# Oneflow-Inc/libai

Measured on AMD Instinct MI355X. Metric: tokens/sec (whole node), GPT-2 345M 3D-parallel at 1/2/4/8 MI355X, higher is better.
Workload: dtype bf16; 1 GPU; model=gpt2-345m (nl24 h1024 nah16 seq1024), global_batch=48, seq_len=1024, parallelism=dp1

## Files before the change

### libai_amd/csrc/kernels/flash_attn.hip

```cpp
#include "common.h"
#include "launchers.h"

#include <type_traits>

namespace {

typedef __bf16 bf16_t;
typedef __bf16 bf16x8_t __attribute__((ext_vector_type(8)));
typedef __bf16 bf16x4_t __attribute__((ext_vector_type(4)));
typedef float f32x16_t __attribute__((ext_vector_type(16)));

#define QB 32
#define NW 4
#define QBLK (QB * NW)
#define KVB 64

#ifdef FLASH_SETPRIO
#define PRIO_HI() __builtin_amdgcn_s_setprio(1)
#define PRIO_LO() __builtin_amdgcn_s_setprio(0)
#else
#define PRIO_HI()
#define PRIO_LO()
#endif

__device__ __forceinline__ uint32_t pack_bf16x2(float lo, float hi) {
  union {
    uint32_t u;
    bf16_t h[2];
  } r;
  r.h[0] = (bf16_t)lo;
  r.h[1] = (bf16_t)hi;
  return r.u;
}

__device__ __forceinline__ float and_f32(float x, uint32_t m) {
  return __uint_as_float(__float_as_uint(x) & m);
}

__device__ __forceinline__ float mul_then_sub(float a, float b, float c) {
#pragma clang fp contract(off)
  return a * b - c;
}

__device__ __forceinline__ bf16x8_t repack_chunk(const float* sv8) {
  uint32_t x0 = pack_bf16x2(sv8[0], sv8[1]);
  uint32_t z0 = pack_bf16x2(sv8[2], sv8[3]);
  uint32_t y0 = pack_bf16x2(sv8[4], sv8[5]);
  uint32_t w0 = pack_bf16x2(sv8[6], sv8[7]);
  auto rx = __builtin_amdgcn_permlane32_swap(x0, y0, false, false);
  auto rz = __builtin_amdgcn_permlane32_swap(z0, w0, false, false);
  uint32_t words[4] = {(uint32_t)rx[0], (uint32_t)rz[0], (uint32_t)rx[1],
                       (uint32_t)rz[1]};
  bf16x8_t out;
  memcpy(&out, words, 16);
  return out;
}


template <int D>
__device__ __forceinline__ void row_img_write(bf16_t* lds, int row, int col8,
                                              bf16x8_t val) {
  int byte = (row * D + col8 * 8) * 2;
  byte ^= (row & 15) << 4;
  *(bf16x8_t*)((char*)lds + byte) = val;
}

template <int D>
__device__ __forceinline__ bf16x8_t row_img_frag(const bf16_t* lds, int row, int c,
                                                 int hi) {
  int byte = (row * D + c * 16 + hi * 8) * 2;
  byte ^= (row & 15) << 4;
  return *(const bf16x8_t*)((const char*)lds + byte);
}

template <int D>
__device__ __forceinline__ void tr_img_write(bf16_t* lds, int row, int d0,
                                             bf16x8_t val) {
  int idx = (((row >> 2) * (D / 16) + (d0 >> 4)) * 64) + (row & 3) * 16 + (d0 & 15);
  *(bf16x8_t*)(lds + idx) = val;
}

template <int D>
__device__ __forceinline__ bf16x8_t tr_img_frag(const bf16_t* lds, int rbase, int dt,
                                                int lane) {
  const int hi = lane >> 5;
  const int l31 = lane & 31;
  const int r0 = rbase + hi * 8;
  const int d0 = dt * 32 + (l31 & ~15);
  const bf16_t* p0 =
      lds + (((r0 >> 2) * (D / 16) + (d0 >> 4)) * 64) + (lane & 15) * 4;
  const bf16_t* p1 =
      lds + ((((r0 + 4) >> 2) * (D / 16) + (d0 >> 4)) * 64) + (lane & 15) * 4;
  bf16x4_t a = __builtin_amdgcn_ds_read_tr16_b64_v4bf16(
      (__attribute__((address_space(3))) bf16x4_t*)p0);
  bf16x4_t b = __builtin_amdgcn_ds_read_tr16_b64_v4bf16(
      (__attribute__((address_space(3))) bf16x4_t*)p1);
  bf16x8_t out;
#pragma unroll
  for (int j = 0; j < 4; ++j) {
    out[j] = a[j];
    out[4 + j] = b[j];
  }
  return out;
}

template <int ROWS, int D, bool ROW_IMG, bool TR_IMG>
__device__ __forceinline__ void stage_tile(bf16_t* row_lds, bf16_t* tr_lds,
                                           const bf16_t* gp, int row0, int bound,
                                           int64_t stride, int tid) {
  constexpr int CHUNKS_TOTAL = ROWS * D / 8;
  constexpr int ITER = CDIV(CHUNKS_TOTAL, 256);
#pragma unroll
  for (int cc = 0; cc < ITER; ++cc) {
    const int flat = tid + cc * 256;
    if (flat >= CHUNKS_TOTAL) break;
    const int row = flat / (D / 8);
    const int col8 = flat % (D / 8);
    const int gr = row0 + row;
    bf16x8_t val =
        (gr < bound) ? *(const bf16x8_t*)(gp + (int64_t)gr * stride + col8 * 8)
                     : bf16x8_t{};
    if (ROW_IMG) row_img_write<D>(row_lds, row, col8, val);
    if (TR_IMG) tr_img_write<D>(tr_lds, row, col8 * 8, val);
  }
}

__device__ __forceinline__ uint32_t drop_hash4(uint64_t seed, uint64_t bh,
                                               int64_t Sq, int64_t Sk4, int q,
                                               int kv4) {
  (void)Sq;
  return rnd_hash2(seed, (uint32_t)q * (uint32_t)Sk4 + (uint32_t)kv4,
                   (uint32_t)bh);
}

__device__ __forceinline__ float drop_keep_byte(uint32_t h4, int kv_lo,
                                                uint32_t thr8, float ks) {
  return (((h4 >> (kv_lo * 8)) & 0xFFu) >= thr8) ? ks : 0.f;
}

__device__ __forceinline__ float drop_keep(uint64_t seed, uint64_t bh, int64_t Sq,
                                           int64_t Sk, int q, int kv, uint32_t thr8,
                                           float ks) {
  uint32_t h = drop_hash4(seed, bh, Sq, Sk >> 2, q, kv >> 2);
  return drop_keep_byte(h, kv & 3, thr8, ks);
}

__device__ __forceinline__ int block_tile() {
  return (int)((blockIdx.x + blockIdx.y) % gridDim.x);
}

__device__ __forceinline__ int doc_lo_load(const int* __restrict__ row, int i,
                                           int S) {
  return min(max(row[min(i, S - 1)], 0), i);
}

__device__ __forceinline__ int doc_hi_load(const int* __restrict__ row, int i,
                                           int S) {
  return min(max(row[min(i, S - 1)], i + 1), S);
}

#define RELB_LOG2E 1.4426950408889634f

__device__ __forceinline__ float relb_load(const float* __restrict__ row, int t,
                                           int n_diag) {
  return row[min(max(t, 0), n_diag - 1)];
}

#define RELB_RING 256

__device__ __forceinline__ void relb_flush(float* ring, float* __restrict__ grow,
                                           int tid, int count, int a0, int t_off,
                                           int n_diag) {
  if (tid < count) {
    const int a = a0 + tid;
    const float g = ring[a & (RELB_RING - 1)];
    ring[a & (RELB_RING - 1)] = 0.f;
    const int t = a + t_off;
    if (g != 0.f && t >= 0 && t < n_diag) atomicAdd(grow + t, g);
  }
}

template <int D, FlashVariant V>
__global__ __launch_bounds__(256, D == 64 ? 3 : 2) void flash_fwd_kernel(
    const bf16_t* __restrict__ q, const bf16_t* __restrict__ k,
    const bf16_t* __restrict__ v, bf16_t* __restrict__ o, float* __restrict__ lse,
    const int* __restrict__ kv_len, int64_t q_sb, int64_t q_ss, int64_t q_sh,
    int64_t k_sb, int64_t k_ss, int64_t k_sh, int64_t v_sb, int64_t v_ss,
    int64_t v_sh, int64_t o_sb, int64_t o_ss, int64_t o_sh, int H, int Sq, int Sk,
    float scale, float p_drop, uint64_t seed, int causal, int kv_group,
    const float* __restrict__ alibi_slopes, int window,
    const float* __restrict__ rel_bias, const int* __restrict__ doc_start) {
  constexpr bool ALIBI = V == FlashVariant::kAlibi,
                 WINDOW = V == FlashVariant::kWindow,
                 RELB = V == FlashVariant::kRelBias, DOCS = V == FlashVariant::kDocs;
  constexpr int DT = D / 32;
  constexpr int KC = D / 16;

  __shared__ __align__(16) bf16_t k_lds[2 * KVB * D];
  __shared__ __align__(16) bf16_t v_lds[2 * KVB * D];
  constexpr int FWD_DIAGS = 2 * KVB + QBLK - 1;
  __shared__ float rb_lds[RELB ? FWD_DIAGS : 1];

  const int tid = threadIdx.x;
  const int wave = tid >> 6;
  const int lane = tid & 63;
  const int l31 = lane & 31;
  const int hi = lane >> 5;

  const int bh = blockIdx.y;
  const int b = bh / H, h = bh % H;
  const int q_block = block_tile() * QBLK;
  const int q_base = __builtin_amdgcn_readfirstlane(q_block + wave * QB);

  const int hk = h / kv_group;
  const bf16_t* qp = q + b * q_sb + h * q_sh;
  const bf16_t* kp = k + b * k_sb + hk * k_sh;
  const bf16_t* vp = v + b * v_sb + hk * v_sh;

  const float qscale = scale * 1.4426950408889634f;
  bf16x8_t qfrag[KC];
  {
    const int qrow = min(q_base + l31, Sq - 1);
#pragma unroll
    for (int c = 0; c < KC; ++c) {
      bf16x8_t raw = *(const bf16x8_t*)(qp + (int64_t)qrow * q_ss + c * 16 + hi * 8);
#pragma unroll
      for (int j = 0; j < 8; ++j) raw[j] = (bf16_t)((float)raw[j] * qscale);
      qfrag[c] = raw;
    }
  }

  f32x16_t oacc[DT];
#pragma unroll
  for (int t = 0; t < DT; ++t) oacc[t] = f32x16_t{};
  float m_run = -3.0e38f, l_run = 0.f;

  const int sk_eff = (kv_len != nullptr) ? kv_len[b] : Sk;
  const int kv_end = causal ? min(sk_eff, q_block + QBLK) : sk_eff;
  const int n_rounds = CDIV(kv_end, 2 * KVB);
  const float ks = (p_drop > 0.f) ? 1.0f / (1.0f - p_drop) : 1.0f;
  const int qg = q_base + l31;
  float slope2 = 0.f;
  if constexpr (ALIBI) slope2 = alibi_slopes[h] * 1.4426950408889634f;

  int round0 = 0;
  if constexpr (WINDOW) round0 = max(0, q_block - window + 1) / (2 * KVB);
  int doc_lo = 0, doc_lo_w = 0, doc_lo_top = 0;
  if constexpr (DOCS) {
    const int* dsp = doc_start + (int64_t)b * Sq;
    doc_lo = doc_lo_load(dsp, qg, Sq);
    round0 = __builtin_amdgcn_readfirstlane(doc_lo_load(dsp, q_block, Sq)) /
             (2 * KVB);
    doc_lo_w = __builtin_amdgcn_readfirstlane(doc_lo_load(dsp, q_base, Sq));
    doc_lo_top =
        __builtin_amdgcn_readfirstlane(doc_lo_load(dsp, q_base + QB - 1, Sq));
  }
  const int n_diag = Sq + Sk - 1;
  const float* rbp = nullptr;
  if constexpr (RELB) rbp = rel_bias + (int64_t)h * n_diag;
  const int rb_lane = (QBLK - 1) - (qg - q_block);

  for (int round = round0; round < n_rounds; ++round) {
    const int kvR = round * 2 * KVB;
    __syncthreads();
    stage_tile<2 * KVB, D, true, false>(k_lds, nullptr, kp, kvR, Sk, k_ss, tid);
    stage_tile<2 * KVB, D, false, true>(nullptr, v_lds, vp, kvR, Sk, v_ss, tid);
    if constexpr (RELB) {
      if (tid < FWD_DIAGS)
        rb_lds[tid] =
            relb_load(rbp, kvR - q_block - (QBLK - 1) + tid + (Sq - 1), n_diag) *
            RELB_LOG2E;
    }
    __syncthreads();

    for (int sub = 0; sub < 2; ++sub) {
    const int kv0 = kvR + sub * KVB;
    const int ro = sub * KVB;
    if (kv0 >= kv_end || (causal && kv0 > q_base + QB - 1)) continue;
    if constexpr (WINDOW) {
      if (kv0 + KVB - 1 < q_base - window + 1) continue;
    }
    if constexpr (DOCS) {
      if (kv0 + KVB - 1 < doc_lo_w) continue;
    }

    f32x16_t s0{}, s1{};
    PRIO_HI();
#pragma unroll
    for (int c = 0; c < KC; ++c) {
      bf16x8_t ka = row_img_frag<D>(k_lds, ro + l31, c, hi);
      s0 = __builtin_amdgcn_mfma_f32_32x32x16_bf16(ka, qfrag[c], s0, 0, 0, 0);
      bf16x8_t kb = row_img_frag<D>(k_lds, ro + l31 + 32, c, hi);
      s1 = __builtin_amdgcn_mfma_f32_32x32x16_bf16(kb, qfrag[c], s1, 0, 0, 0);
    }
    PRIO_LO();

    float sv[2][16];
    bool interior = kv0 + KVB <= sk_eff && q_base + QB <= Sq &&
                    (!causal || q_base >= kv0 + KVB - 1);
    if constexpr (WINDOW) interior = interior && (q_base + QB - 1 - kv0 < window);
    if constexpr (DOCS) interior = interior && (kv0 >= doc_lo_top);
    auto softmax_tile = [&](auto masked_c) {
      constexpr bool MASKED = decltype(masked_c)::value;
      float pmax = -3.0e38f;
      float rel0 = 0.f;
      if constexpr (ALIBI) rel0 = (float)(kv0 + 4 * hi - qg);
#pragma unroll
      for (int r = 0; r < 16; ++r) {
        int kva = kv0 + (r & 3) + 8 * (r >> 2) + 4 * hi;
        int kvb = kva + 32;
        float a = s0[r], bb = s1[r];
        if constexpr (ALIBI) {
          const float off = (float)((r & 3) + 8 * (r >> 2));
          a = fmaf(slope2, rel0 + off, a);
          bb = fmaf(slope2, rel0 + (off + 32.f), bb);
        }
        if constexpr (RELB) {
          const int e = rb_lane + ro + (r & 3) + 8 * (r >> 2) + 4 * hi;
          a += rb_lds[e];
          bb += rb_lds[e + 32];
        }
        if constexpr (MASKED) {
          if (kva >= sk_eff || (causal && kva > qg)) a = -3.0e38f;
          if (kvb >= sk_eff || (causal && kvb > qg)) bb = -3.0e38f;
          if constexpr (WINDOW) {
            if (qg - kva >= window) a = -3.0e38f;
            if (qg - kvb >= window) bb = -3.0e38f;
          }
          if constexpr (DOCS) {
            if (kva < doc_lo) a = -3.0e38f;
            if (kvb < doc_lo) bb = -3.0e38f;
          }
        }
        sv[0][r] = a;
        sv[1][r] = bb;
        pmax = fmaxf(pmax, fmaxf(a, bb));
      }
      pmax = fmaxf(pmax, __shfl_xor(pmax, 32));

      const float m_new = fmaxf(m_run, pmax);
      float alpha = __builtin_amdgcn_exp2f(m_run - m_new);
      if constexpr (MASKED) alpha = (m_run <= -3.0e38f) ? 0.f : alpha;
      m_run = m_new;
      float lsum = 0.f;
#pragma unroll
      for (int t = 0; t < 2; ++t)
#pragma unroll
        for (int r = 0; r < 16; ++r) {
          float e = __builtin_amdgcn_exp2f(sv[t][r] - m_new);
          if constexpr (MASKED) e = (sv[t][r] <= -3.0e38f) ? 0.f : e;
          sv[t][r] = e;
          lsum += e;
        }
      lsum += __shfl_xor(lsum, 32);
      l_run = l_run * alpha + lsum;
      return alpha;
    };
    const float alpha = interior ? softmax_tile(std::false_type{})
                                 : softmax_tile(std::true_type{});
#pragma unroll
    for (int t = 0; t < DT; ++t)
#pragma unroll
      for (int r = 0; r < 16; ++r) oacc[t][r] *= alpha;

    if (p_drop > 0.f) {
      const uint32_t thr8 = drop_threshold_u8(p_drop);
#pragma unroll
      for (int t = 0; t < 2; ++t)
#pragma unroll
        for (int r4 = 0; r4 < 4; ++r4) {
          const int kvb = kv0 + t * 32 + 8 * r4 + 4 * hi;
          const uint32_t h = drop_hash4(seed, bh, Sq, Sk >> 2, qg, kvb >> 2);
#pragma unroll
          for (int j = 0; j < 4; ++j)
            sv[t][r4 * 4 + j] *= drop_keep_byte(h, j, thr8, ks);
        }
    }

    PRIO_HI();
#pragma unroll
    for (int t = 0; t < 2; ++t) {
#pragma unroll
      for (int c16 = 0; c16 < 2; ++c16) {
        bf16x8_t pfrag = repack_chunk(&sv[t][c16 * 8]);
        const int kvc = t * 32 + c16 * 16;
#pragma unroll
        for (int dt = 0; dt < DT; ++dt) {
          bf16x8_t vfrag = tr_img_frag<D>(v_lds, ro + kvc, dt, lane);
          oacc[dt] =
              __builtin_amdgcn_mfma_f32_32x32x16_bf16(vfrag, pfrag, oacc[dt], 0, 0, 0);
        }
      }
    }
    PRIO_LO();
    }
  }

  const float inv_l = (l_run > 0.f) ? 1.0f / l_run : 0.f;
  bf16_t* op = o + b * o_sb + h * o_sh + (int64_t)qg * o_ss;
  if (qg < Sq) {
#pragma unroll
    for (int dt = 0; dt < DT; ++dt)
#pragma unroll
      for (int r4 = 0; r4 < 4; ++r4) {
        bf16x4_t pk;
#pragma unroll
        for (int j = 0; j < 4; ++j) pk[j] = (bf16_t)(oacc[dt][r4 * 4 + j] * inv_l);
        *(bf16x4_t*)(op + dt * 32 + 8 * r4 + 4 * hi) = pk;
      }
    if (hi == 0 && lse != nullptr)
      lse[((int64_t)bh * Sq) + qg] =
          m_run * 0.6931471805599453f + __logf(l_run > 0.f ? l_run : 1.f);
  }
}

template <int D>
__global__ void rowdot_kernel(const bf16_t* __restrict__ dout,
                              const bf16_t* __restrict__ o, float* __restrict__ drow,
                              int64_t sb, int64_t ss, int64_t sh, int H, int Sq,
                              int64_t nrows) {
  constexpr int LPR = D / 8;
  constexpr int RPW = 64 / LPR;
  const int64_t wave_id = ((int64_t)blockIdx.x * blockDim.x + threadIdx.x) / 64;
  const int lane = threadIdx.x & 63;
  const int64_t row = wave_id * RPW + lane / LPR;
  if (row >= nrows) return;
  const int64_t BSH = (int64_t)Sq * H;
  const int64_t b = row / BSH;
  const int64_t rem = row % BSH;
  const int64_t qi = rem / H;
  const int64_t h = rem % H;
  const bf16_t* dp = dout + b * sb + qi * ss + h * sh + (lane % LPR) * 8;
  const bf16_t* op = o + b * sb + qi * ss + h * sh + (lane % LPR) * 8;
  u16x8 dv = *(const u16x8*)dp;
  u16x8 ov = *(const u16x8*)op;
  float s = 0.f;
#pragma unroll
  for (int j = 0; j < 8; ++j) s += bf2f(dv[j]) * bf2f(ov[j]);
#pragma unroll
  for (int off = LPR / 2; off > 0; off >>= 1) s += __shfl_xor(s, off, 64);
  if (lane % LPR == 0) drow[(b * H + h) * Sq + qi] = s;
}

template <int D, FlashVariant V>
__global__ __launch_bounds__(256, 2) void flash_bwd_kv_kernel(
    const bf16_t* __restrict__ q, const bf16_t* __restrict__ k,
    const bf16_t* __restrict__ v, const bf16_t* __restrict__ dout,
    const float* __restrict__ lse, const float* __restrict__ drow,
    const int* __restrict__ kv_len, bf16_t* __restrict__ dk,
    bf16_t* __restrict__ dv, int64_t q_sb, int64_t q_ss,
    int64_t q_sh, int64_t k_sb, int64_t k_ss, int64_t k_sh, int64_t v_sb,
    int64_t v_ss, int64_t v_sh, int64_t do_sb, int64_t do_ss, int64_t do_sh,
    int64_t dk_sb, int64_t dk_ss, int64_t dk_sh, int64_t dv_sb, int64_t dv_ss,
    int64_t dv_sh, int H, int Sq, int Sk, float scale, float p_drop, uint64_t seed,
    int causal, int kv_group, const float* __restrict__ alibi_slopes,
    int window, const float* __restrict__ rel_bias,
    const int* __restrict__ doc_end) {
  constexpr bool ALIBI = V == FlashVariant::kAlibi,
                 WINDOW = V == FlashVariant::kWindow,
                 RELB = V == FlashVariant::kRelBias, DOCS = V == FlashVariant::kDocs;
  constexpr int DT = D / 32;
  constexpr int KC = D / 16;
  constexpr int QTILE = (D == 64) ? 2 * QB : QB;
  constexpr int NSUB = QTILE / QB;
  constexpr int KV_DIAGS = QBLK + QTILE - 1;
  __shared__ float rb_lds[RELB ? KV_DIAGS : 1];

  __shared__ __align__(16) bf16_t q_row[QTILE * D];
  __shared__ __align__(16) bf16_t q_tr[QTILE * D];
  __shared__ __align__(16) bf16_t do_row[QTILE * D];
  __shared__ __align__(16) bf16_t do_tr[QTILE * D];
  __shared__ __align__(16) float lse_lds[QTILE];
  __shared__ __align__(16) float drow_lds[QTILE];
  constexpr bool PIPE = D == 64;

  const int tid = threadIdx.x;
  const int wave = tid >> 6;
  const int lane = tid & 63;
  const int l31 = lane & 31;
  const int hi = lane >> 5;

  const int Hkv = H / kv_group;
  const int bhk = blockIdx.y;
  const int b = bhk / Hkv, hk = bhk % Hkv;
  const int kv_block = block_tile() * QBLK;
  const int kv_base = __builtin_amdgcn_readfirstlane(kv_block + wave * QB);
  const int kvg = kv_base + l31;

  const bf16_t* kp = k + b * k_sb + hk * k_sh;
  const bf16_t* vp = v + b * v_sb + hk * v_sh;

  constexpr bool KV_PERSIST = D == 64;
  const int kvr_ld = min(kvg, Sk - 1);
  auto load_kf = [&](int c) {
    return *(const bf16x8_t*)(kp + (int64_t)kvr_ld * k_ss + c * 16 + hi * 8);
  };
  auto load_vf = [&](int c) {
    return *(const bf16x8_t*)(vp + (int64_t)kvr_ld * v_ss + c * 16 + hi * 8);
  };
  bf16x8_t kf[KV_PERSIST ? KC : 1], vf[KV_PERSIST ? KC : 1];
  if constexpr (KV_PERSIST) {
#pragma unroll
    for (int c = 0; c < KC; ++c) {
      kf[c] = load_kf(c);
      vf[c] = load_vf(c);
    }
  }
  auto get_kf = [&](int c) {
    if constexpr (KV_PERSIST) return kf[c];
    else return load_kf(c);
  };
  auto get_vf = [&](int c) {
    if constexpr (KV_PERSIST) return vf[c];
    else return load_vf(c);
  };

  f32x16_t dk_acc[DT], dv_acc[DT];
#pragma unroll
  for (int t = 0; t < DT; ++t) {
    dk_acc[t] = f32x16_t{};
    dv_acc[t] = f32x16_t{};
  }

  const float ks = (p_drop > 0.f) ? 1.0f / (1.0f - p_drop) : 1.0f;
  const int sk_eff = (kv_len != nullptr) ? kv_len[b] : Sk;
  const int qt_start = causal ? (kv_block / QTILE) : 0;
  int q_hi = Sq;
  if constexpr (WINDOW) q_hi = min(Sq, kv_block + QBLK + window - 1);
  int doc_hi = 0, doc_hi_w = 0, doc_hi_bot = 0;
  if constexpr (DOCS) {
    const int* dep = doc_end + (int64_t)b * Sk;
    doc_hi = doc_hi_load(dep, kvg, Sk);
    const int k_last = max(min(kv_block + QBLK, min(Sk, sk_eff)) - 1, 0);
    q_hi = min(Sq, __builtin_amdgcn_readfirstlane(doc_hi_load(dep, k_last, Sk)));
    doc_hi_w =
        __builtin_amdgcn_readfirstlane(doc_hi_load(dep, kv_base + QB - 1, Sk));
    doc_hi_bot = __builtin_amdgcn_readfirstlane(doc_hi_load(dep, kv_base, Sk));
  }
  const int n_qtiles = (kv_block < sk_eff) ? CDIV(q_hi, QTILE) : 0;

  const uint32_t sk4_mul = (uint32_t)(Sk >> 2) * RND_HASH_LO_MUL;
  const uint32_t hkey_lane =
      (uint32_t)(4 * hi + (l31 & 3)) * sk4_mul +
      (uint32_t)((kv_base + (l31 & ~3)) >> 2) * RND_HASH_LO_MUL;

  for (int g = 0; g < kv_group; ++g) {
  const int h = hk * kv_group + g;
  const int bh = b * H + h;
  const uint32_t hkey_head = (uint32_t)seed ^ ((uint32_t)bh * RND_HASH_HI_MUL) ^
                             (uint32_t)(seed >> 32);
  const bf16_t* qp = q + b * q_sb + h * q_sh;
  const bf16_t* dop = dout + b * do_sb + h * do_sh;
  float slope = 0.f;
  if constexpr (ALIBI) slope = alibi_slopes[h];
  const int n_diag = Sq + Sk - 1;
  const float* rbp = nullptr;
  if constexpr (RELB) rbp = rel_bias + (int64_t)h * n_diag;
  const float* rb_lane = rb_lds + ((QBLK - 1) - (kvg - kv_block) + 4 * hi);

  auto stage_all = [&](int qt) {
    const int q0 = qt * QTILE;
    stage_tile<QTILE, D, true, true>(q_row, q_tr, qp, q0, Sq, q_ss, tid);
    stage_tile<QTILE, D, true, true>(do_row, do_tr, dop, q0, Sq, do_ss, tid);
    if (tid < QTILE) {
      int qr = min(q0 + tid, Sq - 1);
      lse_lds[tid] = lse[(int64_t)bh * Sq + qr];
      drow_lds[tid] = drow[(int64_t)bh * Sq + qr];
    }
    if constexpr (RELB) {
      if (tid < KV_DIAGS)
        rb_lds[tid] = relb_load(
            rbp, kv_block - q0 + (QBLK - 1) - tid + (Sq - 1), n_diag);
    }
  };

  constexpr int PF = QTILE * D / 8 / 256;
  bf16x8_t pf_q[PF], pf_do[PF];
  float pf_lse = 0.f, pf_drow = 0.f, pf_rb = 0.f;
  auto load_tile = [&](int qt) {
    const int q0 = qt * QTILE;
#pragma unroll
    for (int cc = 0; cc < PF; ++cc) {
      const int flat = tid + cc * 256;
      const int gr = q0 + flat / (D / 8);
      const int col8 = flat % (D / 8);
      pf_q[cc] = (gr < Sq)
                     ? *(const bf16x8_t*)(qp + (int64_t)gr * q_ss + col8 * 8)
                     : bf16x8_t{};
      pf_do[cc] = (gr < Sq)
                      ? *(const bf16x8_t*)(dop + (int64_t)gr * do_ss + col8 * 8)
                      : bf16x8_t{};
    }
    if (tid < QTILE) {
      int qr = min(q0 + tid, Sq - 1);
      pf_lse = lse[(int64_t)bh * Sq + qr];
      pf_drow = drow[(int64_t)bh * Sq + qr];
    }
    if constexpr (RELB) {
      if (tid < KV_DIAGS)
        pf_rb = relb_load(
            rbp, kv_block - q0 + (QBLK - 1) - tid + (Sq - 1), n_diag);
    }
  };
  auto write_tile = [&] {
#pragma unroll
    for (int cc = 0; cc < PF; ++cc) {
      const int flat = tid + cc * 256;
      const int row = flat / (D / 8);
      const int col8 = flat % (D / 8);
      row_img_write<D>(q_row, row, col8, pf_q[cc]);
      tr_img_write<D>(q_tr, row, col8 * 8, pf_q[cc]);
      row_img_write<D>(do_row, row, col8, pf_do[cc]);
      tr_img_write<D>(do_tr, row, col8 * 8, pf_do[cc]);
    }
    if (tid < QTILE) {
      lse_lds[tid] = pf_lse;
      drow_lds[tid] = pf_drow;
    }
    if constexpr (RELB) {
      if (tid < KV_DIAGS) rb_lds[tid] = pf_rb;
    }
  };
  auto vm_drain = [] { __builtin_amdgcn_s_waitcnt(0x0F70); };

  auto compute_tile = [&](int q0) {
    if (causal && q0 + QTILE - 1 < kv_base) return;
    if constexpr (WINDOW) {
      if (q0 - (kv_base + QB - 1) >= window) return;
    }
    if constexpr (DOCS) {
      if (q0 >= doc_hi_w) return;
    }

#pragma unroll 1
    for (int sub = 0; sub < NSUB; ++sub) {
      const int q0s = q0 + sub * QB;
      if (causal && q0s + QB - 1 < kv_base) continue;
      if constexpr (WINDOW) {
        if (q0s - (kv_base + QB - 1) >= window) continue;
      }
      if constexpr (DOCS) {
        if (q0s >= doc_hi_w) continue;
      }
      const int ro = sub * QB;

      f32x16_t s{};
      f32x16_t dpd{};
      PRIO_HI();
#pragma unroll
      for (int c = 0; c < KC; ++c) {
        bf16x8_t qa = row_img_frag<D>(q_row, ro + l31, c, hi);
        s = __builtin_amdgcn_mfma_f32_32x32x16_bf16(qa, get_kf(c), s, 0, 0, 0);
        bf16x8_t da = row_img_frag<D>(do_row, ro + l31, c, hi);
        dpd = __builtin_amdgcn_mfma_f32_32x32x16_bf16(da, get_vf(c), dpd, 0, 0, 0);
      }
      PRIO_LO();

      bool interior = q0s + QB <= Sq && kv_base + QB <= sk_eff &&
                      (!causal || q0s >= kv_base + QB - 1);
      if constexpr (WINDOW)
        interior = interior && (q0s + QB - 1 - kv_base < window);
      if constexpr (DOCS) interior = interior && (q0s + QB - 1 < doc_hi_bot);

#pragma unroll
      for (int c16 = 0; c16 < 2; ++c16) {
        float pd8[8], ds8[8];
        auto elems = [&](auto masked_c, auto drop_c) {
        constexpr bool MASKED = decltype(masked_c)::value;
        constexpr bool DROP = decltype(drop_c)::value;
        const uint32_t thr8 = drop_threshold_u8(p_drop);
        const int byte_sh = (l31 & 3) * 8;
#pragma unroll
        for (int r4 = 0; r4 < 2; ++r4) {
          const int qbase = q0s + c16 * 16 + 8 * r4 + 4 * hi;
          const float4 lse4 = *(const float4*)__builtin_assume_aligned(
              &lse_lds[qbase - q0], 16);
          const float4 drow4 = *(const float4*)__builtin_assume_aligned(
              &drow_lds[qbase - q0], 16);
          const float lse_r[4] = {lse4.x, lse4.y, lse4.z, lse4.w};
          const float drow_r[4] = {drow4.x, drow4.y, drow4.z, drow4.w};
          const float* rb_run = rb_lane + (qbase - 4 * hi - q0);
          uint32_t hq = 0;
          if constexpr (DROP)
            hq = rnd_hash_mix(
                hkey_head ^
                (__builtin_amdgcn_readfirstlane(
                     (uint32_t)(q0s + c16 * 16 + 8 * r4) * sk4_mul) +
                 hkey_lane));
          uint32_t hqj[4];
          hqj[0] = (uint32_t)__builtin_amdgcn_mov_dpp((int)hq, 0x00, 0xF, 0xF, true);
          hqj[1] = (uint32_t)__builtin_amdgcn_mov_dpp((int)hq, 0x55, 0xF, 0xF, true);
          hqj[2] = (uint32_t)__builtin_amdgcn_mov_dpp((int)hq, 0xAA, 0xF, 0xF, true);
          hqj[3] = (uint32_t)__builtin_amdgcn_mov_dpp((int)hq, 0xFF, 0xF, 0xF, true);
#pragma unroll
          for (int j = 0; j < 4; ++j) {
            const int k = r4 * 4 + j;
            const int r = c16 * 8 + k;
            const int qrow = qbase + j;
            float x;
            if constexpr (ALIBI)
              x = fmaf(slope, (float)(kvg - qrow), s[r] * scale) - lse_r[j];
            else if constexpr (RELB)
              x = fmaf(s[r], scale, rb_run[j] - lse_r[j]);
            else
              x = fmaf(s[r], scale, -lse_r[j]);
            float keep = 1.f;
            if constexpr (DROP)
              keep = (((hqj[j] >> byte_sh) & 0xFFu) >= thr8) ? ks : 0.f;
            if constexpr (MASKED) {
              bool valid =
                  qrow < Sq && kvg < sk_eff && (!causal || qrow >= kvg);
              if constexpr (WINDOW) valid = valid && (qrow - kvg < window);
              if constexpr (DOCS) valid = valid && (qrow < doc_hi);
              const uint32_t vm = valid ? 0xFFFFFFFFu : 0u;
              const float p = and_f32(__expf(x), vm);
              pd8[k] = p * keep;
              ds8[k] = and_f32(
                  scale * p * mul_then_sub(dpd[r], keep, drow_r[j]), vm);
            } else {
              const float p = __expf(x);
              pd8[k] = p * keep;
              ds8[k] = scale * p * mul_then_sub(dpd[r], keep, drow_r[j]);
            }
          }
        }
        };
        if (p_drop > 0.f) {
          if (interior) elems(std::false_type{}, std::true_type{});
          else elems(std::true_type{}, std::true_type{});
        } else {
          if (interior) elems(std::false_type{}, std::false_type{});
          else elems(std::true_type{}, std::false_type{});
        }
        bf16x8_t pdf = repack_chunk(pd8);
        bf16x8_t dsf = repack_chunk(ds8);
        const int qc = ro + c16 * 16;
        PRIO_HI();
#pragma unroll
        for (int dt = 0; dt < DT; ++dt) {
          bf16x8_t dof = tr_img_frag<D>(do_tr, qc, dt, lane);
          dv_acc[dt] =
              __builtin_amdgcn_mfma_f32_32x32x16_bf16(dof, pdf, dv_acc[dt], 0, 0, 0);
          bf16x8_t qtf = tr_img_frag<D>(q_tr, qc, dt, lane);
          dk_acc[dt] =
              __builtin_amdgcn_mfma_f32_32x32x16_bf16(qtf, dsf, dk_acc[dt], 0, 0, 0);
        }
        PRIO_LO();
      }
    }
  };

  if constexpr (PIPE) {
    if (qt_start < n_qtiles) {
      stage_all(qt_start);
      __syncthreads();
    }
    for (int qt = qt_start; qt < n_qtiles; ++qt) {
      const bool more = qt + 1 < n_qtiles;
      vm_drain();
      if (more) load_tile(qt + 1);
      compute_tile(qt * QTILE);
      __syncthreads();
      if (more) {
        write_tile();
        __syncthreads();
      }
    }
  } else {
    for (int qt = qt_start; qt < n_qtiles; ++qt) {
      __syncthreads();
      stage_all(qt);
      __syncthreads();
      compute_tile(qt * QTILE);
    }
  }

  }

  if (kvg < Sk) {
    bf16_t* dkp = dk + b * dk_sb + hk * dk_sh + (int64_t)kvg * dk_ss;
    bf16_t* dvp = dv + b * dv_sb + hk * dv_sh + (int64_t)kvg * dv_ss;
#pragma unroll
    for (int dt = 0; dt < DT; ++dt)
#pragma unroll
      for (int r4 = 0; r4 < 4; ++r4) {
        bf16x4_t a, c;
#pragma unroll
        for (int j = 0; j < 4; ++j) {
          a[j] = (bf16_t)dk_acc[dt][r4 * 4 + j];
          c[j] = (bf16_t)dv_acc[dt][r4 * 4 + j];
        }
        *(bf16x4_t*)(dkp + dt * 32 + 8 * r4 + 4 * hi) = a;
        *(bf16x4_t*)(dvp + dt * 32 + 8 * r4 + 4 * hi) = c;
      }
  }
}

template <int D, FlashVariant V>
__global__ __launch_bounds__(256, 2) void flash_bwd_q_kernel(
    const bf16_t* __restrict__ q, const bf16_t* __restrict__ k,
    const bf16_t* __restrict__ v, const bf16_t* __restrict__ dout,
    const float* __restrict__ lse, const float* __restrict__ drow,
    const int* __restrict__ kv_len, bf16_t* __restrict__ dq, int64_t q_sb,
    int64_t q_ss, int64_t q_sh, int64_t k_sb,
    int64_t k_ss, int64_t k_sh, int64_t v_sb, int64_t v_ss, int64_t v_sh,
    int64_t do_sb, int64_t do_ss, int64_t do_sh, int64_t dq_sb, int64_t dq_ss,
    int64_t dq_sh, int H, int Sq, int Sk, float scale, float p_drop, uint64_t seed,
    int causal, int kv_group, const float* __restrict__ alibi_slopes,
    int window, const float* __restrict__ rel_bias,
    float* __restrict__ d_rel_bias, const int* __restrict__ doc_start) {
  constexpr bool ALIBI = V == FlashVariant::kAlibi,
                 WINDOW = V == FlashVariant::kWindow,
                 RELB = V == FlashVariant::kRelBias, DOCS = V == FlashVariant::kDocs;
  constexpr int DT = D / 32;
  constexpr int KC = D / 16;
  constexpr int KVTILE = (D == 64) ? 2 * QB : QB;
  constexpr int NSUB = KVTILE / QB;

  __shared__ __align__(16) bf16_t k_row[KVTILE * D];
  __shared__ __align__(16) bf16_t k_tr[KVTILE * D];
  __shared__ __align__(16) bf16_t v_row[KVTILE * D];
  constexpr int Q_DIAGS = KVTILE + QBLK - 1;
  static_assert(Q_DIAGS <= RELB_RING, "a tile's diagonals must fit the ring");
  __shared__ float rb_lds[RELB ? Q_DIAGS : 1];
  __shared__ float drb_lds[RELB ? RELB_RING : 1];

  const int tid = threadIdx.x;
  const int wave = tid >> 6;
  const int lane = tid & 63;
  const int l31 = lane & 31;
  const int hi = lane >> 5;

  const int bh = blockIdx.y;
  const int b = bh / H, h = bh % H;
  const int q_block = block_tile() * QBLK;
  const int q_base = __builtin_amdgcn_readfirstlane(q_block + wave * QB);
  const int qg = q_base + l31;

  const int hk = h / kv_group;
  const bf16_t* qp = q + b * q_sb + h * q_sh;
  const bf16_t* kp = k + b * k_sb + hk * k_sh;
  const bf16_t* vp = v + b * v_sb + hk * v_sh;
  const bf16_t* dop = dout + b * do_sb + h * do_sh;

  const int qr_ld = min(qg, Sq - 1);
  bf16x8_t qf[KC], dof[KC];
#pragma unroll
  for (int c = 0; c < KC; ++c) {
    qf[c] = *(const bf16x8_t*)(qp + (int64_t)qr_ld * q_ss + c * 16 + hi * 8);
    dof[c] = *(const bf16x8_t*)(dop + (int64_t)qr_ld * do_ss + c * 16 + hi * 8);
  }
  const float lse_lane = lse[(int64_t)bh * Sq + min(qg, Sq - 1)];
  const float drow_lane = drow[(int64_t)bh * Sq + min(qg, Sq - 1)];
  float slope = 0.f;
  if constexpr (ALIBI) slope = alibi_slopes[h];

  f32x16_t dq_acc[DT];
#pragma unroll
  for (int t = 0; t < DT; ++t) dq_acc[t] = f32x16_t{};

  const float ks = (p_drop > 0.f) ? 1.0f / (1.0f - p_drop) : 1.0f;
  const int sk_eff = (kv_len != nullptr) ? kv_len[b] : Sk;
  const int kv_end = causal ? min(sk_eff, q_block + QBLK) : sk_eff;
  const int n_tiles = CDIV(kv_end, KVTILE);

  int tile0 = 0;
  if constexpr (WINDOW) tile0 = max(0, q_block - window + 1) / KVTILE;
  int doc_lo = 0, doc_lo_w = 0, doc_lo_top = 0;
  if constexpr (DOCS) {
    const int* dsp = doc_start + (int64_t)b * Sq;
    doc_lo = doc_lo_load(dsp, qg, Sq);
    tile0 = __builtin_amdgcn_readfirstlane(doc_lo_load(dsp, q_block, Sq)) / KVTILE;
    doc_lo_w = __builtin_amdgcn_readfirstlane(doc_lo_load(dsp, q_base, Sq));
    doc_lo_top =
        __builtin_amdgcn_readfirstlane(doc_lo_load(dsp, q_base + QB - 1, Sq));
  }

  const int n_diag = Sq + Sk - 1;
  const float* rbp = nullptr;
  float* drbp = nullptr;
  if constexpr (RELB) {
    rbp = rel_bias + (int64_t)h * n_diag;
    drbp = d_rel_bias + (int64_t)h * n_diag;
    drb_lds[tid] = 0.f;
  }
  const int rb_lane = (QBLK - 1) - (qg - q_block);
  const int rb_t0 = (Sq - 1) - q_block - (QBLK - 1);

  for (int tile = tile0; tile < n_tiles; ++tile) {
    const int kv0 = tile * KVTILE;
    __syncthreads();
    stage_tile<KVTILE, D, true, true>(k_row, k_tr, kp, kv0, Sk, k_ss, tid);
    stage_tile<KVTILE, D, true, false>(v_row, nullptr, vp, kv0, Sk, v_ss, tid);
    if constexpr (RELB) {
      if (tile > tile0)
        relb_flush(drb_lds, drbp, tid, KVTILE, kv0 - KVTILE, rb_t0, n_diag);
      if (tid < Q_DIAGS)
        rb_lds[tid] = relb_load(rbp, kv0 + rb_t0 + tid, n_diag);
    }
    __syncthreads();

    if (causal && kv0 > q_base + QB - 1) continue;

#pragma unroll
    for (int sub = 0; sub < NSUB; ++sub) {
      const int kv0s = kv0 + sub * QB;
      if (kv0s >= kv_end || (causal && kv0s > q_base + QB - 1)) continue;
      if constexpr (WINDOW) {
        if (kv0s + QB - 1 < q_base - window + 1) continue;
      }
      if constexpr (DOCS) {
        if (kv0s + QB - 1 < doc_lo_w) continue;
      }
      const int ro = sub * QB;

      f32x16_t st{};
      f32x16_t dpdt{};
      PRIO_HI();
#pragma unroll
      for (int c = 0; c < KC; ++c) {
        bf16x8_t ka = row_img_frag<D>(k_row, ro + l31, c, hi);
        st = __builtin_amdgcn_mfma_f32_32x32x16_bf16(ka, qf[c], st, 0, 0, 0);
        bf16x8_t va = row_img_frag<D>(v_row, ro + l31, c, hi);
        dpdt = __builtin_amdgcn_mfma_f32_32x32x16_bf16(va, dof[c], dpdt, 0, 0, 0);
      }
      PRIO_LO();

      float ds[16];
      bool interior = kv0s + QB <= sk_eff && q_base + QB <= Sq &&
                      (!causal || q_base >= kv0s + QB - 1);
      if constexpr (WINDOW)
        interior = interior && (q_base + QB - 1 - kv0s < window);
      if constexpr (DOCS) interior = interior && (kv0s >= doc_lo_top);
      auto ds_tile = [&](auto masked_c) {
        constexpr bool MASKED = decltype(masked_c)::value;
        const uint32_t thr8 = drop_threshold_u8(p_drop);
        float rel0 = 0.f;
        if constexpr (ALIBI) rel0 = (float)(kv0s + 4 * hi - qg);
        constexpr bool PRE_REDUCE = D == 64;
        const int slot0 = (rb_lane + kv0s + 4 * hi) & (RELB_RING - 1);
        float g_main = 0.f, g_wrap = 0.f;
        auto diag_add = [&](int r, float gv) {
          const int sh = (r & 3) + 8 * (r >> 2);
          if constexpr (!PRE_REDUCE) {
            atomicAdd(&drb_lds[(slot0 + sh) & (RELB_RING - 1)], gv);
          } else if (sh == 0) {
            g_main = gv;
          } else {
            const float t = __shfl(gv, ((l31 + sh) & 31) | (lane & 32));
            const bool wrapped = l31 + sh >= 32;
            g_main += wrapped ? 0.f : t;
            g_wrap += wrapped ? t : 0.f;
          }
        };
#pragma unroll
        for (int r4 = 0; r4 < 4; ++r4) {
          const int kvb = kv0s + 8 * r4 + 4 * hi;
          const uint32_t h = (p_drop > 0.f)
                                 ? drop_hash4(seed, bh, Sq, Sk >> 2, qg, kvb >> 2)
                                 : 0;
#pragma unroll
          for (int j = 0; j < 4; ++j) {
            const int r = r4 * 4 + j;
            const int kv = kvb + j;
            float x;
            int e = 0;
            if constexpr (RELB) e = rb_lane + (kv - kv0);
            if constexpr (ALIBI)
              x = fmaf(slope, rel0 + (float)(8 * r4 + j), st[r] * scale) - lse_lane;
            else if constexpr (RELB)
              x = fmaf(st[r], scale, rb_lds[e] - lse_lane);
            else
              x = fmaf(st[r], scale, -lse_lane);
            if constexpr (MASKED) {
              bool valid = kv < sk_eff && qg < Sq && (!causal || kv <= qg);
              if constexpr (WINDOW) valid = valid && (qg - kv < window);
              if constexpr (DOCS) valid = valid && (kv >= doc_lo);
              const uint32_t vm = valid ? 0xFFFFFFFFu : 0u;
              float p = and_f32(__expf(x), vm);
              float keep = (p_drop > 0.f) ? drop_keep_byte(h, j, thr8, ks) : 1.f;
              const float sp = scale * p;
              const float dd = fmaf(dpdt[r], keep, -drow_lane);
              ds[r] = and_f32(sp * dd, vm);
              if constexpr (RELB) diag_add(r, and_f32(p * dd, vm));
            } else {
              float p = __expf(x);
              float keep = (p_drop > 0.f) ? drop_keep_byte(h, j, thr8, ks) : 1.f;
              const float sp = scale * p;
              const float dd = fmaf(dpdt[r], keep, -drow_lane);
              ds[r] = sp * dd;
              if constexpr (RELB) diag_add(r, p * dd);
            }
          }
        }
        if constexpr (RELB && PRE_REDUCE) {
          atomicAdd(&drb_lds[slot0], g_main);
          atomicAdd(&drb_lds[(slot0 + 32) & (RELB_RING - 1)], g_wrap);
        }
      };
      if (interior) ds_tile(std::false_type{});
      else ds_tile(std::true_type{});

      PRIO_HI();
#pragma unroll
      for (int c16 = 0; c16 < 2; ++c16) {
        bf16x8_t dsf = repack_chunk(&ds[c16 * 8]);
        const int kvc = ro + c16 * 16;
#pragma unroll
        for (int dt = 0; dt < DT; ++dt) {
          bf16x8_t ktf = tr_img_frag<D>(k_tr, kvc, dt, lane);
          dq_acc[dt] =
              __builtin_amdgcn_mfma_f32_32x32x16_bf16(ktf, dsf, dq_acc[dt], 0, 0, 0);
        }
      }
      PRIO_LO();
    }
  }

  if constexpr (RELB) {
    __syncthreads();
    if (n_tiles > tile0)
      relb_flush(drb_lds, drbp, tid, Q_DIAGS, (n_tiles - 1) * KVTILE, rb_t0,
                 n_diag);
  }

  if (qg < Sq) {
    bf16_t* dqp = dq + b * dq_sb + h * dq_sh + (int64_t)qg * dq_ss;
#pragma unroll
    for (int dt = 0; dt < DT; ++dt)
#pragma unroll
      for (int r4 = 0; r4 < 4; ++r4) {
        bf16x4_t a;
#pragma unroll
        for (int j = 0; j < 4; ++j) a[j] = (bf16_t)dq_acc[dt][r4 * 4 + j];
        *(bf16x4_t*)(dqp + dt * 32 + 8 * r4 + 4 * hi) = a;
      }
  }
}

template <class E>
__global__ void attn_dropout_apply_kernel(typename E::T* __restrict__ x, int64_t BH,
                                          int64_t Sq, int64_t Sk, float p,
                                          float keep_scale, uint64_t seed) {
  const int64_t total = BH * Sq * Sk;
  const uint32_t thr8 = drop_threshold_u8(p);
  for (int64_t i = blockIdx.x * (int64_t)blockDim.x + threadIdx.x; i < total;
       i += (int64_t)gridDim.x * blockDim.x) {
    const int64_t row = i / Sk;
    const int kv = (int)(i % Sk);
    uint32_t h = rnd_hash2(seed, (uint32_t)(row % Sq) * (uint32_t)(Sk >> 2) +
                                     (uint32_t)(kv >> 2),
                           (uint32_t)(row / Sq));
    float kp = drop_keep_byte(h, kv & 3, thr8, keep_scale);
    x[i] = E::from_f(E::to_f(x[i]) * kp);
  }
}

}

static const bf16_t* in(const StridedBSHD& t) { return (const bf16_t*)t.ptr; }
static bf16_t* out(const StridedBSHD& t) { return (bf16_t*)t.ptr; }

static int clamp_window(int window, int Sq, int Sk) {
  return window > 0 ? min(window, max(Sq, Sk)) : 0;
}

extern "C" void flash_fwd_bf16(const FlashFwdArgs& a, hipStream_t stream) {
  const dim3 grid(CDIV(a.Sq, QBLK), a.B * a.H), block(256);
  const int window = clamp_window(a.window, a.Sq, a.Sk);
  const FlashVariant variant =
      flash_variant(a.alibi_slopes, window, a.rel_bias, a.doc_start);
  flash_dispatch(a.D, variant, [&](auto dc, auto vc) {
    flash_fwd_kernel<decltype(dc)::value, decltype(vc)::value>
        <<<grid, block, 0, stream>>>(
            in(a.q), in(a.k), in(a.v), out(a.o), a.lse, a.kv_len,
            a.q.sb, a.q.ss, a.q.sh,
            a.k.sb, a.k.ss, a.k.sh,
            a.v.sb, a.v.ss, a.v.sh,
            a.o.sb, a.o.ss, a.o.sh,
            a.H, a.Sq, a.Sk, a.scale, a.p_drop, a.seed, a.causal, a.kv_group,
            a.alibi_slopes, window, a.rel_bias, a.doc_start);
  });
}

extern "C" void flash_bwd_bf16(const FlashBwdArgs& a, hipStream_t stream) {
  const dim3 block(256);
  const int Hkv = a.H / a.kv_group;
  const dim3 grid_kv(CDIV(a.Sk, QBLK), a.B * Hkv), grid_q(CDIV(a.Sq, QBLK), a.B * a.H);
  const int window = clamp_window(a.window, a.Sq, a.Sk);
  const FlashVariant variant =
      flash_variant(a.alibi_slopes, window, a.rel_bias, a.doc_start);
  const int rpw = 64 / (a.D / 8);
  const int64_t rows = (int64_t)a.B * a.Sq * a.H;
  const uint32_t rowdot_blocks = (uint32_t)CDIV(CDIV(rows, rpw) * 64, 256);
  flash_dispatch(a.D, variant, [&](auto dc, auto vc) {
    constexpr int DD = decltype(dc)::value;
    constexpr FlashVariant VV = decltype(vc)::value;
    rowdot_kernel<DD><<<dim3(rowdot_blocks), 256, 0, stream>>>(
        in(a.dout), in(a.o), a.drow_ws, a.dout.sb, a.dout.ss, a.dout.sh, a.H, a.Sq,
        rows);
    flash_bwd_kv_kernel<DD, VV><<<grid_kv, block, 0, stream>>>(
        in(a.q), in(a.k), in(a.v), in(a.dout), a.lse, a.drow_ws, a.kv_len,
        out(a.dk), out(a.dv),
        a.q.sb, a.q.ss, a.q.sh,
        a.k.sb, a.k.ss, a.k.sh,
        a.v.sb, a.v.ss, a.v.sh,
        a.dout.sb, a.dout.ss, a.dout.sh,
        a.dk.sb, a.dk.ss, a.dk.sh,
        a.dv.sb, a.dv.ss, a.dv.sh,
        a.H, a.Sq, a.Sk, a.scale, a.p_drop, a.seed, a.causal, a.kv_group,
        a.alibi_slopes, window, a.rel_bias, a.doc_end);
    flash_bwd_q_kernel<DD, VV><<<grid_q, block, 0, stream>>>(
        in(a.q), in(a.k), in(a.v), in(a.dout), a.lse, a.drow_ws, a.kv_len,
        out(a.dq),
        a.q.sb, a.q.ss, a.q.sh,
        a.k.sb, a.k.ss, a.k.sh,
        a.v.sb, a.v.ss, a.v.sh,
        a.dout.sb, a.dout.ss, a.dout.sh,
        a.dq.sb, a.dq.ss, a.dq.sh,
        a.H, a.Sq, a.Sk, a.scale, a.p_drop, a.seed, a.causal, a.kv_group,
        a.alibi_slopes, window, a.rel_bias, a.d_rel_bias, a.doc_start);
  });
}

#define ATTN_DROP_LAUNCHER(SUFF, ETYPE)                                            \
  extern "C" void attn_dropout_apply_##SUFF(void* x, int64_t BH, int64_t Sq,       \
                                            int64_t Sk, float p, uint64_t seed,    \
                                            hipStream_t stream) {                  \
    int64_t n = BH * Sq * Sk;                                                      \
    int64_t g = CDIV(n, 256);                                                      \
    if (g > 4096) g = 4096;                                                        \
    attn_dropout_apply_kernel<ETYPE><<<dim3((uint32_t)g), dim3(256), 0, stream>>>( \
        (ETYPE::T*)x, BH, Sq, Sk, p, 1.0f / (1.0f - p), seed);                     \
  }

ATTN_DROP_LAUNCHER(bf16, BF16Elem)
ATTN_DROP_LAUNCHER(f32, F32Elem)
```

Measured before the change: 302,200 tokens/s.

## Restage flash attention KV tiles through registers and raise bwd-q occupancy

Replaces the per-iteration stage_tile calls in the forward and dQ-backward kernels with a register-staged load and write. It uses precomputed swizzled LDS addresses and clamped global row indices in place of branches. The first tile is staged before the loop, and each next tile is staged after the current tile's compute. The dQ backward kernel's launch bounds rise to 3 blocks per CU for D=64 non-relbias variants to increase occupancy, at the cost of register pressure and possible spills. Load and LDS write still run back to back with barriers between them, so global latency is largely not hidden.

```diff
diff --git a/libai_amd/csrc/kernels/flash_attn.hip b/libai_amd/csrc/kernels/flash_attn.hip
--- a/libai_amd/csrc/kernels/flash_attn.hip
+++ b/libai_amd/csrc/kernels/flash_attn.hip
@@ -125,6 +125,52 @@
   }
 }
 
+template <int ROWS, int D>
+struct TileRegs {
+  static constexpr int N = ROWS * D / 8 / 256;
+  static_assert(N * 256 * 8 == ROWS * D, "whole chunks for all 256 threads");
+  bf16x8_t c[N];
+};
+
+template <int ROWS, int D>
+__device__ __forceinline__ void tile_load(TileRegs<ROWS, D>& t, const bf16_t* gp,
+                                          int row0, int bound, int64_t stride,
+                                          int tid) {
+#pragma unroll
+  for (int cc = 0; cc < TileRegs<ROWS, D>::N; ++cc) {
+    const int flat = tid + cc * 256;
+    const int gr = min(row0 + flat / (D / 8), bound - 1);
+    const int col8 = tid % (D / 8);
+    t.c[cc] = *(const bf16x8_t*)(gp + ((int64_t)gr * stride + col8 * 8));
+  }
+}
+
+template <int ROWS, int D, bool ROW_IMG, bool TR_IMG>
+__device__ __forceinline__ void tile_write(bf16_t* row_lds, bf16_t* tr_lds,
+                                           const TileRegs<ROWS, D>& t, int row0,
+                                           int bound, int tid) {
+  constexpr int RPP = 256 / (D / 8);
+  static_assert(RPP % 16 == 0, "swizzle phase must repeat per pass");
+  const int r0 = tid / (D / 8);
+  const int col8 = tid % (D / 8);
+  char* rp = (char*)row_lds + (((r0 * D + col8 * 8) * 2) ^ ((r0 & 15) << 4));
+  bf16_t* tp = tr_lds + (((r0 >> 2) * (D / 16) + (col8 >> 1)) * 64) +
+               (r0 & 3) * 16 + (col8 & 1) * 8;
+#pragma unroll
+  for (int cc = 0; cc < TileRegs<ROWS, D>::N; ++cc) {
+    const bf16x8_t val = (row0 + r0 + cc * RPP < bound) ? t.c[cc] : bf16x8_t{};
+    if (ROW_IMG) *(bf16x8_t*)(rp + cc * RPP * D * 2) = val;
+    if (TR_IMG) *(bf16x8_t*)(tp + cc * (RPP / 4) * (D / 16) * 64) = val;
+  }
+}
+
+__device__ __forceinline__ int stage_tid(int tid) {
+  asm volatile("" : "+v"(tid));
+  return tid;
+}
+
+__device__ __forceinline__ void vm_drain() { __builtin_amdgcn_s_waitcnt(0x0F70); }
+
 __device__ __forceinline__ uint32_t drop_hash4(uint64_t seed, uint64_t bh,
                                                int64_t Sq, int64_t Sk4, int q,
                                                int kv4) {
@@ -260,18 +306,36 @@
   if constexpr (RELB) rbp = rel_bias + (int64_t)h * n_diag;
   const int rb_lane = (QBLK - 1) - (qg - q_block);
 
+  TileRegs<2 * KVB, D> pf_k, pf_v;
+  float pf_rb = 0.f;
+  auto load_round = [&](int rnd) {
+    const int st = stage_tid(tid);
+    tile_load(pf_k, kp, rnd * 2 * KVB, Sk, k_ss, st);
+    if constexpr (RELB)
+      pf_rb = relb_load(
+          rbp, rnd * 2 * KVB - q_block - (QBLK - 1) + st + (Sq - 1), n_diag);
+    tile_load(pf_v, vp, rnd * 2 * KVB, Sk, v_ss, stage_tid(tid));
+  };
+  auto write_round = [&](int rnd) {
+    const int st = stage_tid(tid);
+    tile_write<2 * KVB, D, true, false>(k_lds, nullptr, pf_k, rnd * 2 * KVB, Sk,
+                                        st);
+    tile_write<2 * KVB, D, false, true>(nullptr, v_lds, pf_v, rnd * 2 * KVB, Sk,
+                                        st);
+    if constexpr (RELB) {
+      if (st < FWD_DIAGS) rb_lds[st] = pf_rb * RELB_LOG2E;
+    }
+  };
+  if (round0 < n_rounds) {
+    load_round(round0);
+    write_round(round0);
+    __syncthreads();
+  }
+
   for (int round = round0; round < n_rounds; ++round) {
     const int kvR = round * 2 * KVB;
-    __syncthreads();
-    stage_tile<2 * KVB, D, true, false>(k_lds, nullptr, kp, kvR, Sk, k_ss, tid);
-    stage_tile<2 * KVB, D, false, true>(nullptr, v_lds, vp, kvR, Sk, v_ss, tid);
-    if constexpr (RELB) {
-      if (tid < FWD_DIAGS)
-        rb_lds[tid] =
-            relb_load(rbp, kvR - q_block - (QBLK - 1) + tid + (Sq - 1), n_diag) *
-            RELB_LOG2E;
-    }
-    __syncthreads();
+    const bool more = round + 1 < n_rounds;
+    vm_drain();
 
     for (int sub = 0; sub < 2; ++sub) {
     const int kv0 = kvR + sub * KVB;
@@ -394,6 +458,13 @@
     }
     PRIO_LO();
     }
+
+    __syncthreads();
+    if (more) {
+      load_round(round + 1);
+      write_round(round + 1);
+      __syncthreads();
+    }
   }
 
   const float inv_l = (l_run > 0.f) ? 1.0f / l_run : 0.f;
@@ -621,8 +692,6 @@
       if (tid < KV_DIAGS) rb_lds[tid] = pf_rb;
     }
   };
-  auto vm_drain = [] { __builtin_amdgcn_s_waitcnt(0x0F70); };
-
   auto compute_tile = [&](int q0) {
     if (causal && q0 + QTILE - 1 < kv_base) return;
     if constexpr (WINDOW) {
@@ -797,7 +866,8 @@
 }
 
 template <int D, FlashVariant V>
-__global__ __launch_bounds__(256, 2) void flash_bwd_q_kernel(
+__global__ __launch_bounds__(256, (D == 64 && V != FlashVariant::kRelBias) ? 3 : 2)
+void flash_bwd_q_kernel(
     const bf16_t* __restrict__ q, const bf16_t* __restrict__ k,
     const bf16_t* __restrict__ v, const bf16_t* __restrict__ dout,
     const float* __restrict__ lse, const float* __restrict__ drow,
@@ -887,20 +957,33 @@
   const int rb_lane = (QBLK - 1) - (qg - q_block);
   const int rb_t0 = (Sq - 1) - q_block - (QBLK - 1);
 
+  TileRegs<KVTILE, D> pf_k, pf_v;
+  float pf_rb = 0.f;
+  auto load_tile = [&](int t) {
+    const int st = stage_tid(tid);
+    tile_load(pf_k, kp, t * KVTILE, Sk, k_ss, st);
+    tile_load(pf_v, vp, t * KVTILE, Sk, v_ss, st);
+    if constexpr (RELB)
+      pf_rb = relb_load(rbp, t * KVTILE + rb_t0 + st, n_diag);
+  };
+  auto write_tile = [&](int t) {
+    const int st = stage_tid(tid);
+    tile_write<KVTILE, D, true, true>(k_row, k_tr, pf_k, t * KVTILE, Sk, st);
+    tile_write<KVTILE, D, true, false>(v_row, nullptr, pf_v, t * KVTILE, Sk, st);
+    if constexpr (RELB) {
+      if (st < Q_DIAGS) rb_lds[st] = pf_rb;
+    }
+  };
+  if (tile0 < n_tiles) {
+    load_tile(tile0);
+    write_tile(tile0);
+  }
+  __syncthreads();
+
   for (int tile = tile0; tile < n_tiles; ++tile) {
     const int kv0 = tile * KVTILE;
-    __syncthreads();
-    stage_tile<KVTILE, D, true, true>(k_row, k_tr, kp, kv0, Sk, k_ss, tid);
-    stage_tile<KVTILE, D, true, false>(v_row, nullptr, vp, kv0, Sk, v_ss, tid);
-    if constexpr (RELB) {
-      if (tile > tile0)
-        relb_flush(drb_lds, drbp, tid, KVTILE, kv0 - KVTILE, rb_t0, n_diag);
-      if (tid < Q_DIAGS)
-        rb_lds[tid] = relb_load(rbp, kv0 + rb_t0 + tid, n_diag);
-    }
-    __syncthreads();
-
-    if (causal && kv0 > q_base + QB - 1) continue;
+    const bool more = tile + 1 < n_tiles;
+    vm_drain();
 
 #pragma unroll
     for (int sub = 0; sub < NSUB; ++sub) {
@@ -1015,10 +1098,18 @@
       }
       PRIO_LO();
     }
+
+    __syncthreads();
+    if (more) {
+      if constexpr (RELB)
+        relb_flush(drb_lds, drbp, tid, KVTILE, kv0, rb_t0, n_diag);
+      load_tile(tile + 1);
+      write_tile(tile + 1);
+      __syncthreads();
+    }
   }
 
   if constexpr (RELB) {
-    __syncthreads();
     if (n_tiles > tile0)
       relb_flush(drb_lds, drbp, tid, Q_DIAGS, (n_tiles - 1) * KVTILE, rb_t0,
                  n_diag);
```

After: 305,600 tokens/s (median of 6 runs). 1.01x the previous value.
